# cbacary/MoDeGPT

Measured on AMD Instinct MI355X. Metric: transformer layers compressed/sec (covariance+decomp+rebuild), Llama-3-8B @30%, higher is better.
Workload: dtype f64 from int8 MFMA digit planes, exact route: nine plane pairs + fp64 remainder sums, nothing truncated (error <= 5e-15 per call: fp64 rounding)

## Files before the change

### modegpt_amd/csrc/cov_i8.hip

```cpp
#include <algorithm>
#include <map>
#include <mutex>
#include <tuple>
#include <vector>

#include "common.hpp"
#include <atomic>

namespace mdg {
namespace {

typedef int i32x4 __attribute__((ext_vector_type(4)));
typedef int i32x16 __attribute__((ext_vector_type(16)));

constexpr int NP = 6;
constexpr int TI = 128;
constexpr int KS = 32;
constexpr int PA = TI * KS;
constexpr int FLUSH_STEPS = 2047;
constexpr int TOP_SHIFT = 8 * NP - 10;

constexpr int NSTAT = 8;
constexpr int STAT_D0D1 = 6, STAT_COUNTS = 7;
constexpr int EMAX_COLUMN_OUT = 0x100;

__device__ __forceinline__ void bf16_parts(unsigned b, int& sig, int& ee) {
  const int e = (b >> 7) & 0xFF, m = b & 0x7F;
  sig = e ? (128 | m) : m;
  ee = e ? e : 1;
  if (b & 0x8000) sig = -sig;
}

__global__ __launch_bounds__(256) void i8_colmax_kernel(const bf16_t* x, int64_t ld, int64_t T, int n, int64_t rows_per_block,
                                                        int* emax) {
  const int j = blockIdx.x * 64 + (threadIdx.x & 63);
  const int64_t t0 = (int64_t)blockIdx.y * rows_per_block + (threadIdx.x >> 6);
  const int64_t t1 = min(T, (int64_t)(blockIdx.y + 1) * rows_per_block);
  int best = 1;
  if (j < n)
    for (int64_t t = t0; t < t1; t += 4) {
      int sig, ee;
      bf16_parts(x[t * ld + j], sig, ee);
      if (sig != 0) best = max(best, ee);
    }
  if (j < n) atomicMax(emax + j, best);
}

__device__ __forceinline__ unsigned write_piece_mask(const unsigned (&any)[NP], unsigned char* zmask, int64_t index) {
  unsigned byte = 0;
#pragma unroll
  for (int s = 0; s < NP; s++) {
    const unsigned long long b = __ballot(any[s] != 0);
    const unsigned half = (threadIdx.x & 32) ? (unsigned)(b >> 32) : (unsigned)b;
    byte |= (half != 0) << s;
  }
  if ((threadIdx.x & 31) == 0) zmask[index] = (unsigned char)byte;
  return byte;
// ... 43 lines not shown
          N = (N - d[s]) >> 8;
        }
        d[0] = (int)N;
        dig[0][qq >> 2] |= (unsigned)(d[0] & 255) << (8 * (qq & 3));
#pragma unroll
        for (int s = 0; s < NP; s++) q[s] += d[s] * d[s];
        q[STAT_D0D1] += d[0] * d[1];
      }
#pragma unroll
      for (int s = 0; s < NP; s++) {
        signed char* piece = planes + ((s * groups + G) * (int64_t)nk + kt) * 1024;
        *(i32x4*)(piece + h * 512 + r * 16) = (i32x4){(int)dig[s][0], (int)dig[s][1], (int)dig[s][2], (int)dig[s][3]};
        any[s] |= dig[s][0] | dig[s][1] | dig[s][2] | dig[s][3];
      }
    }
    write_piece_mask(any, zmask, (int64_t)kt * groups + G);
  }
#pragma unroll
  for (int i = 0; i < NSTAT; i++)
    if (q[i]) atomicAdd(&st_lds[i][r], (unsigned long long)q[i]);
  __syncthreads();
  for (int i = threadIdx.x; i < NSTAT * 32; i += 256)
    if (st_lds[i >> 5][i & 31]) atomicAdd(stats + (int64_t)(i >> 5) * n + G * 32 + (i & 31), st_lds[i >> 5][i & 31]);
}

__device__ __forceinline__ int bf16_ee_if_nonzero(unsigned b) {
  const int e = (b >> 7) & 0xFF;
  return (b & 0x7FFF) ? (e ? e : 1) : 0;
}

#ifndef MDG_COLMAX_WGS
#define MDG_COLMAX_WGS 4096
#endif
__global__ __launch_bounds__(256) void i8_colmax_vec_kernel(const bf16_t* x, int64_t ld, int64_t T, int64_t rows_per_block, int* emax) {
  __shared__ int best_lds[128];
  const int cg = threadIdx.x & 15, tl = threadIdx.x >> 4;
  const int j0 = blockIdx.x * 128 + cg * 8;
  const int64_t t0 = (int64_t)blockIdx.y * rows_per_block + tl;
  const int64_t t1 = min(T, (int64_t)(blockIdx.y + 1) * rows_per_block);
  if (threadIdx.x < 128) best_lds[threadIdx.x] = 1;
  __syncthreads();
  int best[8] = {1, 1, 1, 1, 1, 1, 1, 1};
  for (int64_t t = t0; t < t1; t += 16) {
    const i32x4 v = *(const i32x4*)(x + t * ld + j0);
#pragma unroll
    for (int q = 0; q < 4; q++) {
      const unsigned w = (unsigned)v[q];
      best[2 * q] = max(best[2 * q], bf16_ee_if_nonzero(w & 0xFFFF));
      best[2 * q + 1] = max(best[2 * q + 1], bf16_ee_if_nonzero(w >> 16));
    }
  }
#pragma unroll
  for (int q = 0; q < 8; q++) atomicMax(&best_lds[cg * 8 + q], best[q]);
  __syncthreads();
  if (threadIdx.x < 128) atomicMax(emax + blockIdx.x * 128 + threadIdx.x, best_lds[threadIdx.x]);
}

constexpr int SPLIT_TILES = 8;
__global__ __launch_bounds__(256) void i8_split_vec_kernel(const bf16_t* x, int64_t ld, int64_t T, int n, int nk, const int* emax,
                                                           signed char* planes, unsigned long long* stats, unsigned char* zmask) {
  __shared__ __attribute__((aligned(16))) bf16_t tile[64 * 128];
  __shared__ int st_lds[NSTAT + 1][128];
  const int f0 = blockIdx.x * 128;
  const int f = threadIdx.x & 127, ks = threadIdx.x >> 7;
  const int E = emax[f0 + f];
  const int64_t groups = n / 32;
  const int G = (f0 + f) >> 5, r = f & 31;
  for (int i = threadIdx.x; i < (NSTAT + 1) * 128; i += 256) (&st_lds[0][0])[i] = 0;
  int q[NSTAT + 1] = {};
  auto load_tile = [&](int tile_index, i32x4 (&v)[4]) {
    const int64_t tok0 = (int64_t)tile_index * 2 * KS;
#pragma unroll
    for (int c4 = 0; c4 < 4; c4++) {
      const int c = threadIdx.x + 256 * c4;
      const int64_t t = tok0 + (c >> 4);
      v[c4] = (i32x4)0;
      if (t < T) v[c4] = *(const i32x4*)(x + t * ld + f0 + (c & 15) * 8);
    }
  };
  const int tile0 = blockIdx.y * SPLIT_TILES, tiles = (nk + 1) / 2;
  for (int it = 0; it < SPLIT_TILES && tile0 + it < tiles; it++) {
    __syncthreads();
    {
      i32x4 v[4];
      load_tile(tile0 + it, v);
#pragma unroll
      for (int c4 = 0; c4 < 4; c4++) *(i32x4*)(tile + (threadIdx.x + 256 * c4) * 8) = v[c4];
    }
    __syncthreads();
    const int kt = (tile0 + it) * 2 + ks;
    if (kt >= nk) continue;
    unsigned any[NP] = {};
    unsigned deep_dig[2][NP - ALWAYS_WRITTEN_PLANES][4];
#pragma unroll
    for (int h = 0; h < 2; h++) {
      unsigned dig[NP][4];
// ... 98 lines not shown
#pragma unroll
    for (int t = 0; t < NP; t++)
      if (s + t >= P) {
        if (s == t) sq += A[s] * A[t];
        else x += A[s] * A[t];
      }
}
__device__ __forceinline__ double route_violation(const double (&A)[NVAL], int P, double tau_x) {
  double sq, x;
  route_terms(A, P, sq, x);
  return fmax(sq / TAU_SQ, x / tau_x);
}

struct Top2 { double m1; int a1; double m2; };
__device__ __forceinline__ void top2_merge(Top2& a, const Top2& b) {
  if (b.m1 > a.m1 || (b.m1 == a.m1 && b.a1 < a.a1)) {
    a.m2 = fmax(a.m1, b.m2);
    a.m1 = b.m1;
    a.a1 = b.a1;
  } else {
    a.m2 = fmax(a.m2, b.m1);
  }
}

struct RoutePartial {
  Top2 top[NVAL];
  unsigned long long cls[NVAL][64];
  unsigned min_nnz;
};
struct RouteScratch {
  int ticket, forced;
};

__global__ __launch_bounds__(ROUTE_THREADS) void i8_route_kernel(const unsigned long long* __restrict__ stats, int* emax, int n, int64_t n_tokens,
                                                                 double* __restrict__ vals, RoutePartial* partial, RouteScratch* scratch,
                                                                 int* flag, RouteOut* out, int* route_counts, double tolerance) {
  __shared__ unsigned long long group_max[NVAL][64];
  __shared__ Top2 wave_top[ROUTE_THREADS / 64][NVAL];
  __shared__ Top2 top[NVAL];
  __shared__ double floor_of[NVAL];
  __shared__ int decision;
  __shared__ int forced_total, my_ticket;
  __shared__ unsigned min_nnz;
  __shared__ double tau_x_shared;
  const int tid = threadIdx.x, lane = tid & 63, wave = tid >> 6;
  for (int i = tid; i < NVAL * 64; i += ROUTE_THREADS) (&group_max[0][0])[i] = 0ull;
  if (tid == 0) min_nnz = 0xffffffffu;
  __syncthreads();
  auto reduce_top = [&](Top2 (&t)[NVAL]) {
#pragma unroll
    for (int i = 0; i < NVAL; i++) {
#pragma unroll
      for (int off = 32; off >= 1; off >>= 1) {
        Top2 o;
        o.m1 = __shfl_xor(t[i].m1, off);
        o.a1 = __shfl_xor(t[i].a1, off);
        o.m2 = __shfl_xor(t[i].m2, off);
        top2_merge(t[i], o);
      }
      if (lane == 0) wave_top[wave][i] = t[i];
    }
    __syncthreads();
    if (tid < NVAL) {
      Top2 r = wave_top[0][tid];
      for (int w = 1; w < ROUTE_THREADS / 64; w++) top2_merge(r, wave_top[w][tid]);
      top[tid] = r;
    }
    __syncthreads();
  };
// ... 11 lines not shown
      const int ex = emax[j];
      const double nnz = (double)(unsigned)counts, rounded = (double)(unsigned)(counts >> 32);
      const double hi2 = 65536.0 * q[0] + 512.0 * q[STAT_D0D1] + q[1];
      const double norm = (sqrt(fmax(hi2, 0.0)) - 0.5 * sqrt(nnz)) * 4294967296.0;
      const double inv = nnz > 0 ? (norm > 0 ? 1.0 / norm : 1e300) : 0.0;
      double a[NVAL];
#pragma unroll
      for (int s2 = 0; s2 < NP; s2++) a[s2] = q[s2] > 0 ? sqrt(q[s2]) * ldexp(1.0, 8 * (NP - 1 - s2)) * inv : 0.0;
      a[6] = rounded > 0 ? 0.5 * sqrt(rounded) * inv : 0.0;
      nonfinite = (ex & 255) == 255;
      if ((unsigned)counts) atomicMin(&min_nnz, (unsigned)counts);
#pragma unroll
      for (int i = 0; i < NVAL; i++) {
        vals[(int64_t)i * n + j] = a[i];
        if (!nonfinite) t[i] = Top2{a[i], j, -1.0};
      }
      if (nonfinite) emax[j] = ex | EMAX_COLUMN_OUT;
    }
#pragma unroll
    for (int i = 0; i < NVAL; i++)
      if (t[i].m1 > 0.0) atomicMax(&group_max[i][lane], (unsigned long long)__double_as_longlong(t[i].m1));
    const unsigned long long nf = __ballot(nonfinite);
    if (lane == 0 && nf) atomicAdd(&scratch->forced, __popcll(nf));
  }
  reduce_top(t);
  RoutePartial& mine = partial[blockIdx.x];
  if (tid < NVAL) mine.top[tid] = top[tid];
  if (tid == 0) mine.min_nnz = min_nnz;
  for (int i = tid; i < NVAL * 64; i += ROUTE_THREADS) (&mine.cls[0][0])[i] = (&group_max[0][0])[i];
  __threadfence();
  __syncthreads();
  if (tid == 0) my_ticket = atomicAdd(&scratch->ticket, 1);
  __syncthreads();
  if (my_ticket != (int)gridDim.x - 1) return;
  __threadfence();
  const unsigned nwg = gridDim.x;
  if (tid < NVAL) {
    Top2 r = partial[0].top[tid];
    unsigned w = 1;
    for (; w + 4 <= nwg; w += 4) {
      const Top2 b0 = partial[w].top[tid], b1 = partial[w + 1].top[tid], b2 = partial[w + 2].top[tid], b3 = partial[w + 3].top[tid];
      top2_merge(r, b0); top2_merge(r, b1); top2_merge(r, b2); top2_merge(r, b3);
    }
    for (; w < nwg; w++) top2_merge(r, partial[w].top[tid]);
    r.m1 = fmax(r.m1, 0.0);
    r.m2 = fmax(r.m2, 0.0);
    top[tid] = r;
  }
  for (int i = tid; i < NVAL * 64; i += ROUTE_THREADS) {
    unsigned long long m = 0ull;
    unsigned w = 0;
    for (; w + 4 <= nwg; w += 4) {
      const unsigned long long v0 = (&partial[w].cls[0][0])[i], v1 = (&partial[w + 1].cls[0][0])[i], v2 = (&partial[w + 2].cls[0][0])[i],
                               v3 = (&partial[w + 3].cls[0][0])[i];
      m = max(max(m, v0), max(max(v1, v2), v3));
    }
    for (; w < nwg; w++) m = max(m, (&partial[w].cls[0][0])[i]);
    (&group_max[0][0])[i] = m;
  }
  if (tid == 0) {
    forced_total = scratch->forced;
    unsigned m = 0xffffffffu;
    unsigned w = 0;
    for (; w + 4 <= nwg; w += 4) {
      const unsigned v0 = partial[w].min_nnz, v1 = partial[w + 1].min_nnz, v2 = partial[w + 2].min_nnz, v3 = partial[w + 3].min_nnz;
      m = min(min(m, v0), min(min(v1, v2), v3));
    }
    for (; w < nwg; w++) m = min(m, partial[w].min_nnz);
    tau_x_shared = tau_x_of(min(n_tokens, (int64_t)m));
// ... 92 lines not shown
            for (int i = 0; i < NVAL; i++) A2[i] = top[i].a1 == c ? top[i].m2 : top[i].m1;
            const double v = route_violation(A2, P, tau_x);
            if (v < best_v) { best_v = v; best = c; }
          }
          if (best < 0) decision = 1;
          else {
            emax[best] |= EMAX_COLUMN_OUT;
            out->out[n_out] = best;
          }
        }
      }
      __syncthreads();
      const int dec = decision;
      __syncthreads();
      if (dec == 0) return;
      if (dec == 1) break;
      n_out++;
      top_valid = false;
    }
    if (n_out > n_forced) {
      for (int j = tid; j < n; j += ROUTE_THREADS)
        if ((emax[j] & EMAX_COLUMN_OUT) && (emax[j] & 255) != 255) emax[j] &= 255;
      top_valid = false;
      __syncthreads();
    }
  }
  if (tid == 0) {
    out->planes = 0; out->n_out = 0; out->sq = out->x = out->rho = 0.0;
    atomicOr(flag, 2);
  }
  for (int j = tid; j < n; j += ROUTE_THREADS) emax[j] &= 255;
}

__global__ __launch_bounds__(256) void i8_clear_columns_kernel(const RouteOut* route, const int* flag, const int* emax, signed char* planes,
                                                               unsigned char* zmask, int n, int nk) {
  if ((*flag & 2) || (int)blockIdx.x >= route->n_out) return;
  const int j = route->out[blockIdx.x];
  const int64_t groups = n / 32;
  const int G = j >> 5, lane = threadIdx.x & 63, row = lane & 31;
  const bool row_out = (emax[G * 32 + row] & EMAX_COLUMN_OUT) != 0;
  for (int kt = blockIdx.y * 4 + (threadIdx.x >> 6); kt < nk; kt += gridDim.y * 4) {
    const unsigned old_mask = zmask[(int64_t)kt * groups + G];
    unsigned new_mask = 0;
#pragma unroll
    for (int s = 0; s < NP; s++) {
      if (s >= ALWAYS_WRITTEN_PLANES && (old_mask >> s) == 0) continue;
      i32x4* p = (i32x4*)(planes + ((s * groups + G) * (int64_t)nk + kt) * 1024) + lane;
      i32x4 v = *p;
      if (row_out) {
        v = (i32x4)0;
        *p = v;
      }
      if (__ballot((v[0] | v[1] | v[2] | v[3]) != 0)) new_mask |= 1u << s;
    }
    if (lane == 0) zmask[(int64_t)kt * groups + G] = (unsigned char)new_mask;
  }
}

template <int V> struct ic { static constexpr int value = V; };

struct SyrkProblem {
  const signed char* planes;
  const int* emax;
  const unsigned char* zmask;
  double* sigma;
  int64_t ld_sigma;
  int n, block;
};
constexpr int MAX_PROBLEMS = 4;
constexpr int CODE_PROB = 28, CODE_BI = 14;

struct SyrkArgs {
  SyrkProblem prob[MAX_PROBLEMS];
  int nprob, nk;
  unsigned long long* mfma_count;
  const int* route_flag;
  int* route_counts;
  const int2* sched;
  int ngroups;
  double* partial;
  const int4* tail;
  int* xcd_arrive;
  const int* exact_state;
#ifdef MDG_I8_STAMPS
  unsigned long long* stamps;
#endif
#ifdef MDG_I8_WGTIMES
  unsigned long long* wgtimes;
#endif
};
__device__ __forceinline__ int launch_route(const SyrkArgs& a, int& live, int& fallbacks) {
  int six = 0;
  live = fallbacks = 0;
  for (int p = 0; p < a.nprob; p++) {
    const int f = a.route_flag[p];
    if (f & 2) fallbacks++;
    else {
      live++;
      six |= f & 1;
    }
  }
  return live ? six : -1;
// ... 427 lines not shown

constexpr int COMBINE_ELEMS = 1024;
template <int P>
__global__ __launch_bounds__(256) void i8_tail_combine_kernel(SyrkArgs a, int n_tail) {
  constexpr int TJ = wide_tile(P) ? 128 : 64;
  constexpr int PARTS = TI * TJ / COMBINE_ELEMS;
  int live, fallbacks;
  if (!product_launch_runs<P>(a, live, fallbacks)) return;
  const int4 t = a.tail[blockIdx.x / PARTS];
  if (a.route_flag[t.x >> CODE_PROB] & 2) return;
  const SyrkProblem& pr = a.prob[t.x >> CODE_PROB];
  const int bi = (t.x >> CODE_BI) & ((1 << CODE_BI) - 1), bj = t.x & ((1 << CODE_BI) - 1), Q = t.y;
  const double* part = a.partial + (int64_t)t.z * TI * TJ;
#pragma unroll
  for (int i = 0; i < COMBINE_ELEMS / 256; i++) {
    const int e = (blockIdx.x % PARTS) * COMBINE_ELEMS + i * 256 + threadIdx.x;
    const int row = bi * TI + e / TJ, col = bj * TJ + e % TJ;
    if (col > row) continue;
    double* p = pr.sigma + (int64_t)row * pr.ld_sigma + col - (pr.block ? bi * TI : 0);
    double v = *p;
    for (int q = 0; q < Q; q++) v += part[(int64_t)q * TI * TJ + e];
    *p = v;
  }
}

constexpr int COLK_GROUP = 8, COLK_CHUNKS = 64, COLK_WG_COLS = 512, COLK_STAGE = 64, COLK_BATCH = 8;
struct ColArgs {
  const bf16_t* x;
  int64_t ld, T;
  int n, vec;
  const RouteOut* route;
  const int* flag;
  double* part;
};
__device__ __forceinline__ double bf16_bits_to_f64(unsigned b) { return (double)__uint_as_float(b << 16); }

__global__ __launch_bounds__(64) void i8_columns_kernel(ColArgs a) {
  const int pass = blockIdx.z;
  const int n_out = a.route->n_out;
  if ((*a.flag & 2) || pass * COLK_GROUP >= n_out) return;
  const int nj = min(COLK_GROUP, n_out - pass * COLK_GROUP);
  __shared__ __attribute__((aligned(16))) double xj[COLK_STAGE][COLK_GROUP];
  const int lane = threadIdx.x;
  const int my_k = lane % COLK_GROUP;
  const int my_col = my_k < nj ? a.route->out[pass * COLK_GROUP + my_k] : -1;
  const int c0 = blockIdx.x * COLK_WG_COLS + lane * 8;
  const bool active = c0 < a.n;
  const int64_t chunk_len = (a.T + COLK_CHUNKS - 1) / COLK_CHUNKS;
  const int64_t t0 = blockIdx.y * chunk_len, t1 = min(a.T, t0 + chunk_len);
  const unsigned short* xs = (const unsigned short*)a.x;
  auto fetch_group = [&](int64_t t, unsigned short (&g)[COLK_STAGE / 8]) {
#pragma unroll
    for (int i = 0; i < COLK_STAGE / 8; i++) {
      const int64_t tok = t + lane / COLK_GROUP + 8 * i;
      g[i] = (my_col >= 0 && tok < t1) ? xs[tok * a.ld + my_col] : (unsigned short)0;
    }
  };
  double acc[COLK_GROUP][8] = {};
  unsigned short g[COLK_STAGE / 8];
  if (t0 < t1) fetch_group(t0, g);
  for (int64_t t = t0; t < t1; t += COLK_STAGE) {
    __syncthreads();
#pragma unroll
    for (int i = 0; i < COLK_STAGE / 8; i++) xj[lane / COLK_GROUP + 8 * i][my_k] = bf16_bits_to_f64(g[i]);
    __syncthreads();
    if (t + COLK_STAGE < t1) fetch_group(t + COLK_STAGE, g);
    if (!active) continue;
    const int steps = (int)min((int64_t)COLK_STAGE, t1 - t);
    for (int tb = 0; tb < steps; tb += COLK_BATCH) {
      unsigned w[COLK_BATCH][4];
#pragma unroll
      for (int i = 0; i < COLK_BATCH; i++) {
        const bool live = t + tb + i < t1;
// ... 4 lines not shown
        } else {
#pragma unroll
          for (int h = 0; h < 4; h++) w[i][h] = xs[tok * a.ld + c0 + 2 * h] | ((unsigned)xs[tok * a.ld + c0 + 2 * h + 1] << 16);
        }
        if (!live) w[i][0] = w[i][1] = w[i][2] = w[i][3] = 0u;
      }
#pragma unroll
      for (int i = 0; i < COLK_BATCH; i++) {
        double xc[8];
#pragma unroll
        for (int h = 0; h < 4; h++) {
          xc[2 * h] = bf16_bits_to_f64(w[i][h] & 0xFFFFu);
          xc[2 * h + 1] = bf16_bits_to_f64(w[i][h] >> 16);
        }
#pragma unroll
        for (int k = 0; k < COLK_GROUP; k++) {
          const double xk = xj[tb + i][k];
#pragma unroll
          for (int c = 0; c < 8; c++) acc[k][c] += xk * xc[c];
        }
      }
    }
  }
  if (!active) return;
#pragma unroll
  for (int k = 0; k < COLK_GROUP; k++)
    if (k < nj) {
      double* o = a.part + ((int64_t)(pass * COLK_GROUP + k) * COLK_CHUNKS + blockIdx.y) * a.n + c0;
#pragma unroll
      for (int c = 0; c < 8; c++) o[c] = acc[k][c];
    }
}

__global__ __launch_bounds__(256) void i8_columns_reduce_kernel(ColArgs a, const int* emax, double* sigma, int64_t ld_sigma, int block) {
  const int k = blockIdx.y;
  if ((*a.flag & 2) || k >= a.route->n_out) return;
  const int c = blockIdx.x * 256 + threadIdx.x;
  if (c >= a.n) return;
  const int j = a.route->out[k];
  if (block && c / block != j / block) return;
  if ((emax[c] & EMAX_COLUMN_OUT) && c < j) return;
  double v = 0.0;
  for (int q = 0; q < COLK_CHUNKS; q++) v += a.part[((int64_t)k * COLK_CHUNKS + q) * a.n + c];
  const int row = max(c, j), col = min(c, j);
  sigma[(int64_t)row * ld_sigma + col - (block ? row / block * block : 0)] += v;
}


constexpr int LO_CHUNK_STEPS = 64;
constexpr int LO_CAP = 128;
constexpr double LO_ROUND = 8421504.0 / 16777216.0;
constexpr int EXACT_OVERFLOW = 16, EXACT_RAN = 17, EXACT_MODE = 18;
#ifndef MDG_LO_SPARSE_MEAN
#define MDG_LO_SPARSE_MEAN 32
#endif
#ifndef MDG_LO_SPARSE_MAX
#define MDG_LO_SPARSE_MAX 256
#endif
constexpr int LO_SPARSE_MAX = MDG_LO_SPARSE_MAX;
constexpr int LO_SUB = 4, LO_RCAP = 8 * LO_SPARSE_MAX;
constexpr int LO_TILE = 128, LO_PITCH = LO_TILE + 1;

struct __attribute__((aligned(16))) LoEntry {
  double v;
  unsigned off, aux;
};
struct LoProblem {
  const bf16_t* x;
// ... 553 lines not shown
  Schedule sch;
  if (Q >= 2) {
    for (size_t i = 0; i < whole_groups; i++) emit(groups[i]);
    const int pieces = R * Q, tail_rounds = (pieces + 255) / 256;
    std::vector<int2> last((size_t)tail_rounds * 256, make_int2(-1, 0));
    for (int t = 0; t < R; t++) {
      tail.push_back(make_int4(rest[t], Q, t * Q, 0));
      for (int q = 0; q < Q; q++) {
        const int piece = t * Q + q, idx = piece % 256;
        last[(size_t)(piece / 256) * 256 + (idx % 8) * 32 + idx / 8] = make_int2(rest[t], (piece << 10) | (Q << 5) | q);
      }
    }
    table.insert(table.end(), last.begin(), last.end());
    sch.n_tail = (int)tail.size();
    sch.pieces = pieces;
  } else {
    for (auto& g : groups) emit(g);
  }
  sch.ngroups = (int)(table.size() / 32);
  if (hipMalloc((void**)&sch.dev, table.size() * sizeof(int2)) != hipSuccess) return nullptr;
  if (hipMemcpy(sch.dev, table.data(), table.size() * sizeof(int2), hipMemcpyHostToDevice) != hipSuccess) return nullptr;
  if (!tail.empty()) {
    if (hipMalloc((void**)&sch.tail, tail.size() * sizeof(int4)) != hipSuccess) return nullptr;
    if (hipMemcpy(sch.tail, tail.data(), tail.size() * sizeof(int4), hipMemcpyHostToDevice) != hipSuccess) return nullptr;
  }
  return &cache.emplace(key, sch).first->second;
}

constexpr size_t SHARED_BYTES = 256;
struct ProblemWs {
  size_t planes, ints, vals, route, colpart, zmask, lo_entries, lo_counts, lo_xd, lo_rentries, lo_rtotals;
};
int lo_chunks(int64_t T) { return (int)ceil_div(ceil_div(T, (int64_t)KS), (int64_t)LO_CHUNK_STEPS); }
size_t layout(int count, const mdg_cov_problem* pr, ProblemWs* out, size_t* fallback_off) {
  size_t off = SHARED_BYTES + PARTIAL_BYTES, fb = 0;
  for (int i = 0; i < count; i++) {
    const int64_t cols = pr[i].n_feat * pr[i].batch;
    ProblemWs w;
    w.planes = off;
    off += align_up(planes_bytes(pr[i].n_tokens, cols), 256);
    w.ints = off;
    off += align_up(ints_bytes(cols), 256);
    w.vals = off;
    off += align_up((size_t)(NVAL * cols) * sizeof(double) + (size_t)ceil_div(cols, (int64_t)ROUTE_THREADS) * sizeof(RoutePartial), 256);
    w.route = off;
    off += align_up(sizeof(RouteOut), 256);
    w.colpart = off;
    off += align_up((size_t)ROUTE_JMAX * COLK_CHUNKS * (size_t)cols * sizeof(double), 256);
    w.zmask = off;
    off += zmask_bytes(pr[i].n_tokens, cols);
    w.lo_entries = off = align_up(off, 256);
    off += (size_t)cols * lo_chunks(pr[i].n_tokens) * LO_CAP * sizeof(LoEntry);
    w.lo_counts = off;
    off += align_up((size_t)cols * (lo_chunks(pr[i].n_tokens) + 1) * sizeof(int), 256);
    w.lo_xd = off;
    off += align_up((size_t)cols * (size_t)pr[i].n_tokens * sizeof(bf16_t), 256);
    w.lo_rentries = off;
    off += (size_t)(cols / 32) * LO_SUB * LO_RCAP * sizeof(LoEntry);
    w.lo_rtotals = off;
    off += align_up((size_t)(cols / 32) * LO_SUB * sizeof(int), 256);
    if (out) out[i] = w;
    fb = std::max(fb, mdg_cov_accum_ws_bytes(pr[i].n_tokens, pr[i].n_feat, pr[i].batch));
  }
  if (fallback_off) *fallback_off = off;
  return off + fb + 256;
}

bool problems_ok(int count, const mdg_cov_problem* pr) {
  if (count < 1 || count > MAX_PROBLEMS || !pr) return false;
  for (int i = 0; i < count; i++) {
    if (pr[i].n_tokens != pr[0].n_tokens || pr[i].n_tokens < 0 || pr[i].n_tokens >= (1ll << 28) || pr[i].n_feat <= 0 || pr[i].batch < 1) return false;
    if (pr[i].batch == 1 ? pr[i].n_feat % TI != 0 : pr[i].n_feat != TI) return false;
    if (pr[i].n_feat * pr[i].batch >= (1 << 21)) return false;
    if (pr[i].ld < pr[i].n_feat * pr[i].batch || pr[i].ld_sigma < pr[i].n_feat) return false;
    if (pr[i].batch > 1 && (pr[i].ld_sigma != TI || pr[i].sigma_batch_stride != (int64_t)TI * TI)) return false;
// ... 17 lines not shown
  if (have_dev) (void)hipSetDevice(dev0);
  (void)hipGetLastError();
  return rc;
}
}

using namespace mdg;

extern "C" size_t mdg_cov_accum_i8_multi_ws_bytes(int count, const mdg_cov_problem* problems) {
  if (!problems_ok(count, problems) || problems[0].n_tokens == 0) return 0;
  return layout(count, problems, nullptr, nullptr);
}

extern "C" int mdg_cov_accum_i8_multi(int count, const mdg_cov_problem* problems, void* ws, size_t ws_bytes, double tolerance, int flags,
                                      int* used_i8, int* route_counts, void* ev_start, void* ev_stop, void* stream) {
  MDG_CLEAR();
  if (used_i8) *used_i8 = 0;
  MDG_CHECK_ARG(tolerance >= 1.0 && tolerance <= 1e6, "mdg_cov_accum_i8_multi: tolerance factor %g outside [1, 1e6] (1 = guaranteed <= 1.1e-11)",
                tolerance);
  MDG_CHECK_ARG((flags & ~(MDG_I8_NO_EXACT | MDG_I8_EXACT_ALWAYS)) == 0 && flags != (MDG_I8_NO_EXACT | MDG_I8_EXACT_ALWAYS),
                "mdg_cov_accum_i8_multi: bad flags 0x%x", flags);
  bool offer_exact = !(flags & MDG_I8_NO_EXACT);
  for (int i = 0; i < count; i++)
    if ((uint64_t)problems[i].n_tokens * (uint64_t)problems[i].ld * 2ull >= (1ull << 32)) offer_exact = false;
  MDG_CHECK_ARG(problems_ok(count, problems),
                "mdg_cov_accum_i8_multi: 1..%d statistics of the same token count; full ones need n_feat %% 128 == 0, per-head ones "
                "head_dim 128 with contiguous [heads][128][128] sigma; leading dimensions at least the widths (use mdg_cov_accum)",
                MAX_PROBLEMS);
  const int64_t n_tokens = problems[0].n_tokens;
  if (n_tokens == 0) return MDG_OK;
  for (int i = 0; i < count; i++) MDG_CHECK_ARG(problems[i].x && problems[i].sigma, "mdg_cov_accum_i8_multi: null pointer");
  ProblemWs pw[MAX_PROBLEMS];
  size_t fb_off = 0;
  const size_t need = layout(count, problems, pw, &fb_off);
  MDG_CHECK_ARG(ws && ws_bytes >= need, "mdg_cov_accum_i8_multi: workspace %zu < required %zu", ws_bytes, need);
  hipStream_t st = (hipStream_t)stream;
  const int nk = (int)ceil_div(n_tokens, KS);
  int* flag = (int*)ws;
  int* pflag = flag + 12;
  unsigned long long* mfma_count = (unsigned long long*)(flag + 2);
  double* partial = (double*)((char*)ws + SHARED_BYTES);
  void* fb_ws = (char*)ws + fb_off;
  MDG_HIP(hipMemsetAsync(flag, 0, SHARED_BYTES, st));
  SyrkArgs a;
  a.nprob = count;
  a.nk = nk;
  std::vector<std::pair<int, int>> shapes;
  for (int i = 0; i < count; i++) {
    const mdg_cov_problem& q = problems[i];
    const int n = (int)(q.n_feat * q.batch);
    signed char* planes = (signed char*)ws + pw[i].planes;
    int* emax = (int*)((char*)ws + pw[i].ints);
    unsigned long long* stats = (unsigned long long*)(emax + (n + 1) / 2 * 2);
    unsigned char* zmask = (unsigned char*)ws + pw[i].zmask;
    MDG_HIP(hipMemsetAsync(emax, 0, ints_bytes(n), st));
    const bool vec = ((uintptr_t)q.x % 16 == 0) && (q.ld % 8 == 0);
    const int64_t rows_per_block = 2048;
    if (vec) {
      const int64_t slabs = std::min(ceil_div(n_tokens, (int64_t)64), std::max((int64_t)1, (int64_t)MDG_COLMAX_WGS / (n / 128)));
      const int64_t rows_vec = ceil_div(ceil_div(n_tokens, slabs), (int64_t)16) * 16;
      hipLaunchKernelGGL(i8_colmax_vec_kernel, dim3((unsigned)(n / 128), (unsigned)ceil_div(n_tokens, rows_vec)), dim3(256), 0,
                         st, (const bf16_t*)q.x, q.ld, n_tokens, rows_vec, emax);
      hipLaunchKernelGGL(i8_split_vec_kernel, dim3((unsigned)(n / 128), (unsigned)ceil_div(nk, 2 * SPLIT_TILES)), dim3(256), 0, st,
                         (const bf16_t*)q.x, q.ld, n_tokens, n, nk, emax, planes, stats, zmask);
    } else {
      hipLaunchKernelGGL(i8_colmax_kernel, dim3((unsigned)ceil_div(n, 64), (unsigned)ceil_div(n_tokens, rows_per_block)), dim3(256),
                         0, st, (const bf16_t*)q.x, q.ld, n_tokens, n, rows_per_block, emax);
      hipLaunchKernelGGL(i8_split_kernel, dim3((unsigned)(n / 32), (unsigned)ceil_div(nk, SPLIT_STEPS)), dim3(256), 0, st,
                         (const bf16_t*)q.x, q.ld, n_tokens, n, nk, emax, planes, stats, zmask);
    }
    {
      double* vals = (double*)((char*)ws + pw[i].vals);
      RoutePartial* partial = (RoutePartial*)(vals + (size_t)NVAL * n);
      RouteScratch* scratch = (RouteScratch*)(stats + (size_t)NSTAT * n);
      hipLaunchKernelGGL(i8_route_kernel, dim3((unsigned)ceil_div(n, ROUTE_THREADS)), dim3(ROUTE_THREADS), 0, st, stats, emax, n,
                         n_tokens, vals, partial, scratch, pflag + i, (RouteOut*)((char*)ws + pw[i].route), route_counts,
                         tolerance);
    }
    hipLaunchKernelGGL(i8_clear_columns_kernel, dim3(ROUTE_JMAX, (unsigned)std::min(64, (nk + 3) / 4)), dim3(256), 0, st,
                       (const RouteOut*)((char*)ws + pw[i].route), pflag + i, emax, planes, zmask, n, nk);
    MDG_LAUNCH_CHECK();
    a.prob[i] = SyrkProblem{planes, emax, zmask, q.sigma, q.ld_sigma, n, q.batch > 1 ? TI : 0};
    shapes.emplace_back(n / TI, q.batch > 1 ? TI : 0);
  }
  for (int i = count; i < MAX_PROBLEMS; i++) a.prob[i] = a.prob[0];
  a.mfma_count = mfma_count;
  a.route_flag = pflag; a.route_counts = route_counts;
  a.xcd_arrive = flag + 4;
  LoArgs lo;
  a.exact_state = nullptr;
  if (offer_exact) {
    lo.nprob = count;
    lo.nk = nk;
    lo.nch = lo_chunks(n_tokens);
    lo.route_flag = pflag;
    lo.state = flag;
    lo.always = (flags & MDG_I8_EXACT_ALWAYS) ? 1 : 0;
    lo.n_tokens = n_tokens;
    int tiles[3] = {0, 0, 0}, max_groups = 0;
    for (int i = 0; i < count; i++) {
      const mdg_cov_problem& q = problems[i];
      const int n = (int)(q.n_feat * q.batch);
      LoProblem& l = lo.prob[i];
      l.x = (const bf16_t*)q.x; l.ld = q.ld;
      l.planes = a.prob[i].planes; l.zmask = a.prob[i].zmask; l.emax = a.prob[i].emax;
      l.entries = (LoEntry*)((char*)ws + pw[i].lo_entries);
      l.xd = (bf16_t*)((char*)ws + pw[i].lo_xd);
      l.rentries = (LoEntry*)((char*)ws + pw[i].lo_rentries);
      l.rtotals = (int*)((char*)ws + pw[i].lo_rtotals);
      l.pairs = ((uintptr_t)q.x % 4 == 0) && (q.ld % 2 == 0);
      l.counts = (int*)((char*)ws + pw[i].lo_counts);
      l.sigma = q.sigma; l.ld_sigma = q.ld_sigma;
      l.n = n; l.block = q.batch > 1 ? TI : 0;
      const int nG = n / LW_GROUP, per = LW_BLOCK / LW_GROUP;
      for (int tr = 0; tr < 2; tr++) {
        l.tile0[tr] = tiles[tr];
        if (q.batch > 1) {
          tiles[tr] += nG;
        } else {
          for (int P = 0; P * per < nG; P++) tiles[tr] += tr ? std::min(nG, per * (P + 1)) : nG - per * P;
        }
      }
      l.tile0[2] = tiles[2];
      const int rbi = n / TI;
      tiles[2] += q.batch > 1 ? rbi : rbi * (rbi + 1) / 2;
      max_groups = std::max(max_groups, n / 32);
    }
    for (int i = count; i < MAX_PROBLEMS; i++) lo.prob[i] = lo.prob[0];
    for (int k = 0; k < 3; k++) lo.tiles[k] = tiles[k];
    hipLaunchKernelGGL(i8_extract_lo_kernel, dim3((unsigned)max_groups, (unsigned)lo.nch, (unsigned)count), dim3(64), 0, st, lo);
    hipLaunchKernelGGL(i8_compact_lo_kernel, dim3((unsigned)(max_groups * 32), (unsigned)count), dim3(64), 0, st, lo);
    hipLaunchKernelGGL(i8_lo_mode_kernel, dim3(1), dim3(1024), 0, st, lo);
    hipLaunchKernelGGL(i8_residue_lo_kernel, dim3((unsigned)(max_groups * LO_SUB), (unsigned)count), dim3(64), 0, st, lo);
    hipLaunchKernelGGL(i8_copy_xd_kernel, dim3(2048u, (unsigned)count), dim3(256), 0, st, lo);
    hipLaunchKernelGGL(i8_patch_xd_kernel, dim3((unsigned)(max_groups * 32), (unsigned)count), dim3(64), 0, st, lo);
    MDG_LAUNCH_CHECK();
    a.exact_state = flag + EXACT_OVERFLOW;
  }
#ifdef MDG_I8_STAMPS
  static unsigned long long* stamps_dev = nullptr;
  const size_t stamps_n = (size_t)STAMP_WGS * NW * 8;
  if (!stamps_dev) MDG_HIP(hipMalloc(&stamps_dev, stamps_n * 8));
  MDG_HIP(hipMemsetAsync(stamps_dev, 0, stamps_n * 8, st));
  a.stamps = stamps_dev;
#endif
#ifdef MDG_I8_WGTIMES
  static unsigned long long* wg_dev = nullptr;
  if (!wg_dev) MDG_HIP(hipMalloc(&wg_dev, 256 * 64 * 8));
  MDG_HIP(hipMemsetAsync(wg_dev, 0, 256 * 64 * 8, st));
  a.wgtimes = wg_dev;
#endif
  const int n = a.prob[0].n;
  const int rb = n / TI;
  const Schedule* sched_of[2] = {nullptr, nullptr};
  if (rb >= PERSISTENT_MIN_ROWS || count > 1 || problems[0].batch > 1) {
    int dev = 0, n_cu = 0;
    MDG_HIP(hipGetDevice(&dev));
    MDG_HIP(hipDeviceGetAttribute(&n_cu, hipDeviceAttributeMultiprocessorCount, dev));
    if (n_cu == 256)
      for (int i = 0; i < 2; i++) sched_of[i] = schedule_for(shapes, i + 1);
  }
  MDG_CHECK_ARG((count == 1 && problems[0].batch == 1) || (sched_of[0] && sched_of[1]),
                "mdg_cov_accum_i8_multi: several statistics in one launch, and per-head statistics, need the persistent launch (a "
                "256-CU device); use mdg_cov_accum_i8 per full statistic and mdg_cov_accum for the per-head ones");
  {
    size_t zero_bytes = 0;
    for (int i = 0; i < 2; i++)
      if (sched_of[i]) zero_bytes = std::max(zero_bytes, (size_t)sched_of[i]->pieces * TI * (i == 0 ? 128 : 64) * sizeof(double));
    if (zero_bytes) MDG_HIP(hipMemsetAsync(partial, 0, zero_bytes, st));
  }
  a.partial = partial;
  if (ev_start) MDG_HIP(hipEventRecord((hipEvent_t)ev_start, st));
  for (int planes_used : {3, 5, 6}) {
    if (planes_used == 3 && !offer_exact) continue;
    const bool wide = wide_tile(planes_used);
    const int tj = wide ? 128 : 64;
    const size_t lds = (size_t)ring_depth(planes_used) * steps_per_stage(planes_used) * planes_used * (PA + tj * KS);
    const int si = planes_used == 6 ? SB6 : SB5;
    const int sr = (rb + si - 1) / si, nsb = sr * (sr + 1) / 2;
    const int tps = wide ? si * si : 2 * si * si;
    dim3 grid((unsigned)((nsb + 7) / 8 * 8 * tps));
    const Schedule* sch = sched_of[wide ? 0 : 1];
    a.sched = nullptr;
    a.tail = nullptr;
    a.ngroups = 0;
    if (sch) {
      a.sched = sch->dev;
      a.tail = sch->tail;
      a.ngroups = sch->ngroups;
      grid = dim3(256);
    }
    if (planes_used == 3) {
      MDG_HIP(hipFuncSetAttribute((const void*)i8_syrk_kernel<3>, hipFuncAttributeMaxDynamicSharedMemorySize, (int)lds));
      hipLaunchKernelGGL((i8_syrk_kernel<3>), grid, dim3(64 * NW), lds, st, a);
      if (sch && sch->n_tail) hipLaunchKernelGGL((i8_tail_combine_kernel<3>), dim3(sch->n_tail * (TI * tj / COMBINE_ELEMS)), dim3(256), 0, st, a, sch->n_tail);
    } else if (planes_used == 6) {
      MDG_HIP(hipFuncSetAttribute((const void*)i8_syrk_kernel<6>, hipFuncAttributeMaxDynamicSharedMemorySize, (int)lds));
      hipLaunchKernelGGL((i8_syrk_kernel<6>), grid, dim3(64 * NW), lds, st, a);
      if (sch && sch->n_tail) hipLaunchKernelGGL((i8_tail_combine_kernel<6>), dim3(sch->n_tail * (TI * tj / COMBINE_ELEMS)), dim3(256), 0, st, a, sch->n_tail);
    } else {
      MDG_HIP(hipFuncSetAttribute((const void*)i8_syrk_kernel<5>, hipFuncAttributeMaxDynamicSharedMemorySize, (int)lds));
      hipLaunchKernelGGL((i8_syrk_kernel<5>), grid, dim3(64 * NW), lds, st, a);
      if (sch && sch->n_tail) hipLaunchKernelGGL((i8_tail_combine_kernel<5>), dim3(sch->n_tail * (TI * tj / COMBINE_ELEMS)), dim3(256), 0, st, a, sch->n_tail);
    }
    MDG_LAUNCH_CHECK();
  }
  if (ev_stop) MDG_HIP(hipEventRecord((hipEvent_t)ev_stop, st));
  if (offer_exact) {
    const size_t lds = (size_t)LO_TILE * LO_PITCH * sizeof(double);
    MDG_HIP(hipFuncSetAttribute((const void*)i8_lo_product_kernel, hipFuncAttributeMaxDynamicSharedMemorySize, (int)lds));
    hipLaunchKernelGGL(i8_lo_product_kernel, dim3((unsigned)lo.tiles[2]), dim3(LO_THREADS), lds, st, lo);
    hipLaunchKernelGGL(i8_lo_wide_kernel<false>, dim3((unsigned)lo.tiles[0]), dim3(LO_THREADS), 0, st, lo);
    hipLaunchKernelGGL(i8_lo_wide_kernel<true>, dim3((unsigned)lo.tiles[1]), dim3(LO_THREADS), 0, st, lo);
    MDG_LAUNCH_CHECK();
  }
  for (int i = 0; i < count; i++) {
    const mdg_cov_problem& q = problems[i];
    const int n = (int)(q.n_feat * q.batch);
    ColArgs c;
    c.x = (const bf16_t*)q.x; c.ld = q.ld; c.T = n_tokens; c.n = n;
    c.vec = ((uintptr_t)q.x % 16 == 0) && (q.ld % 8 == 0);
    c.route = (const RouteOut*)((char*)ws + pw[i].route);
    c.flag = pflag + i;
    c.part = (double*)((char*)ws + pw[i].colpart);
    hipLaunchKernelGGL(i8_columns_kernel, dim3((unsigned)ceil_div(n, COLK_WG_COLS), COLK_CHUNKS, ROUTE_JMAX / COLK_GROUP), dim3(64), 0, st, c);
    hipLaunchKernelGGL(i8_columns_reduce_kernel, dim3((unsigned)ceil_div(n, 256), ROUTE_JMAX), dim3(256), 0, st, c, a.prob[i].emax, q.sigma,
                       q.ld_sigma, q.batch > 1 ? TI : 0);
    MDG_LAUNCH_CHECK();
  }
  for (int i = 0; i < count; i++) {
    const mdg_cov_problem& q = problems[i];
    const int fb = cov_accum_gated(q.x, MDG_BF16, n_tokens, q.n_feat, q.batch, q.ld, 0, q.sigma, q.ld_sigma, q.sigma_batch_stride, fb_ws,
                                   ws_bytes - fb_off, pflag + i, 2, 2, stream);
    if (fb != MDG_OK) return fb;
  }
#ifdef MDG_I8_STAMPS
  {
    static unsigned long long host[STAMP_WGS * NW * 8];
    MDG_HIP(hipMemcpyAsync(host, a.stamps, sizeof(host), hipMemcpyDeviceToHost, st));
    MDG_HIP(hipStreamSynchronize(st));
    double sum[2][6] = {};
    long cnt[2] = {};
    for (int w = 0; w < STAMP_WGS * NW; w++) {
      const unsigned long long* o = host + (size_t)w * 8;
      if (!o[6]) continue;
      const int role = (w % NW) >= NW / 2;
      for (int i = 0; i < 6; i++) sum[role][i] += (double)o[i] / (double)o[6];
      cnt[role]++;
    }
    for (int role = 0; role < 2; role++)
      if (cnt[role])
        fprintf(stderr, "[stamps n=%d] waves %s: per k-step cycles (s_memtime): wait+barrier %.0f  refill-first %.0f  reads+mfma-issue %.0f  "
                        "wait+refill-last %.0f  | whole tile / nk %.0f  mfma/step %.1f  (%ld waves)\n", n, role ? "4-7" : "0-3",
                sum[role][0] / cnt[role], sum[role][1] / cnt[role], sum[role][2] / cnt[role], sum[role][3] / cnt[role],
                sum[role][4] / cnt[role], sum[role][5] / cnt[role], cnt[role]);
  }
#endif
#ifdef MDG_I8_WGTIMES
  {
    static unsigned long long host[256 * 64];
// ... 103 lines not shown
```

Before: 1.178.

## Batch per-problem preprocessing kernels into single multi-problem launches and merge memsets

```diff
diff --git a/modegpt_amd/csrc/cov_i8.hip b/modegpt_amd/csrc/cov_i8.hip
--- a/modegpt_amd/csrc/cov_i8.hip
+++ b/modegpt_amd/csrc/cov_i8.hip
@@ -23,6 +23,35 @@
 constexpr int NSTAT = 8;
 constexpr int STAT_D0D1 = 6, STAT_COUNTS = 7;
 constexpr int EMAX_COLUMN_OUT = 0x100;
+constexpr int MAX_PROBLEMS = 4;
+
+struct RouteOut;
+struct RoutePartial;
+struct RouteScratch;
+struct CallProblem {
+  const bf16_t* x;
+  int64_t ld;
+  int n, cb0;
+  int* emax;
+  unsigned long long* stats;
+  signed char* planes;
+  unsigned char* zmask;
+  double* vals;
+  RoutePartial* rpartial;
+  RouteScratch* scratch;
+  RouteOut* route;
+  int* flag;
+};
+struct CallArgs {
+  CallProblem prob[MAX_PROBLEMS];
+  int nprob, nk;
+  int64_t T;
+};
+__device__ __forceinline__ int call_problem_of_block(const CallArgs& a, int cb) {
+  int p = 0;
+  while (p + 1 < a.nprob && cb >= a.prob[p + 1].cb0) p++;
+  return p;
+}
 
 __device__ __forceinline__ void bf16_parts(unsigned b, int& sig, int& ee) {
   const int e = (b >> 7) & 0xFF, m = b & 0x7F;
@@ -132,10 +161,14 @@
 #ifndef MDG_COLMAX_WGS
 #define MDG_COLMAX_WGS 4096
 #endif
-__global__ __launch_bounds__(256) void i8_colmax_vec_kernel(const bf16_t* x, int64_t ld, int64_t T, int64_t rows_per_block, int* emax) {
+__global__ __launch_bounds__(256) void i8_colmax_vec_kernel(CallArgs a, int64_t rows_per_block) {
+  const CallProblem& pr = a.prob[call_problem_of_block(a, blockIdx.x)];
+  const bf16_t* x = pr.x;
+  const int64_t ld = pr.ld, T = a.T;
+  const int cb = blockIdx.x - pr.cb0;
   __shared__ int best_lds[128];
   const int cg = threadIdx.x & 15, tl = threadIdx.x >> 4;
-  const int j0 = blockIdx.x * 128 + cg * 8;
+  const int j0 = cb * 128 + cg * 8;
   const int64_t t0 = (int64_t)blockIdx.y * rows_per_block + tl;
   const int64_t t1 = min(T, (int64_t)(blockIdx.y + 1) * rows_per_block);
   if (threadIdx.x < 128) best_lds[threadIdx.x] = 1;
@@ -153,15 +186,22 @@
 #pragma unroll
   for (int q = 0; q < 8; q++) atomicMax(&best_lds[cg * 8 + q], best[q]);
   __syncthreads();
-  if (threadIdx.x < 128) atomicMax(emax + blockIdx.x * 128 + threadIdx.x, best_lds[threadIdx.x]);
+  if (threadIdx.x < 128) atomicMax(pr.emax + cb * 128 + threadIdx.x, best_lds[threadIdx.x]);
 }
 
 constexpr int SPLIT_TILES = 8;
-__global__ __launch_bounds__(256) void i8_split_vec_kernel(const bf16_t* x, int64_t ld, int64_t T, int n, int nk, const int* emax,
-                                                           signed char* planes, unsigned long long* stats, unsigned char* zmask) {
+__global__ __launch_bounds__(256) void i8_split_vec_kernel(CallArgs a) {
+  const CallProblem& pr = a.prob[call_problem_of_block(a, blockIdx.x)];
+  const bf16_t* x = pr.x;
+  const int64_t ld = pr.ld, T = a.T;
+  const int n = pr.n, nk = a.nk;
+  const int* emax = pr.emax;
+  signed char* planes = pr.planes;
+  unsigned long long* stats = pr.stats;
+  unsigned char* zmask = pr.zmask;
   __shared__ __attribute__((aligned(16))) bf16_t tile[64 * 128];
   __shared__ int st_lds[NSTAT + 1][128];
-  const int f0 = blockIdx.x * 128;
+  const int f0 = (blockIdx.x - pr.cb0) * 128;
   const int f = threadIdx.x & 127, ks = threadIdx.x >> 7;
   const int E = emax[f0 + f];
   const int64_t groups = n / 32;
@@ -326,9 +366,19 @@
   int ticket, forced;
 };
 
-__global__ __launch_bounds__(ROUTE_THREADS) void i8_route_kernel(const unsigned long long* __restrict__ stats, int* emax, int n, int64_t n_tokens,
-                                                                 double* __restrict__ vals, RoutePartial* partial, RouteScratch* scratch,
-                                                                 int* flag, RouteOut* out, int* route_counts, double tolerance) {
+__global__ __launch_bounds__(ROUTE_THREADS) void i8_route_kernel(CallArgs a, int* route_counts, double tolerance) {
+  const CallProblem& pr = a.prob[blockIdx.y];
+  const int n = pr.n;
+  const unsigned nwg = (unsigned)((n + ROUTE_THREADS - 1) / ROUTE_THREADS);
+  if (blockIdx.x >= nwg) return;
+  const int64_t n_tokens = a.T;
+  const unsigned long long* __restrict__ stats = pr.stats;
+  int* emax = pr.emax;
+  double* __restrict__ vals = pr.vals;
+  RoutePartial* partial = pr.rpartial;
+  RouteScratch* scratch = pr.scratch;
+  int* flag = pr.flag;
+  RouteOut* out = pr.route;
   __shared__ unsigned long long group_max[NVAL][64];
   __shared__ Top2 wave_top[ROUTE_THREADS / 64][NVAL];
   __shared__ Top2 top[NVAL];
@@ -406,9 +456,8 @@
   __syncthreads();
   if (tid == 0) my_ticket = atomicAdd(&scratch->ticket, 1);
   __syncthreads();
-  if (my_ticket != (int)gridDim.x - 1) return;
+  if (my_ticket != (int)nwg - 1) return;
   __threadfence();
-  const unsigned nwg = gridDim.x;
   if (tid < NVAL) {
     Top2 r = partial[0].top[tid];
     unsigned w = 1;
@@ -567,9 +616,14 @@
   for (int j = tid; j < n; j += ROUTE_THREADS) emax[j] &= 255;
 }
 
-__global__ __launch_bounds__(256) void i8_clear_columns_kernel(const RouteOut* route, const int* flag, const int* emax, signed char* planes,
-                                                               unsigned char* zmask, int n, int nk) {
-  if ((*flag & 2) || (int)blockIdx.x >= route->n_out) return;
+__global__ __launch_bounds__(256) void i8_clear_columns_kernel(CallArgs a) {
+  const CallProblem& pr = a.prob[blockIdx.z];
+  const RouteOut* route = pr.route;
+  const int* emax = pr.emax;
+  signed char* planes = pr.planes;
+  unsigned char* zmask = pr.zmask;
+  const int n = pr.n, nk = a.nk;
+  if ((*pr.flag & 2) || (int)blockIdx.x >= route->n_out) return;
   const int j = route->out[blockIdx.x];
   const int64_t groups = n / 32;
   const int G = j >> 5, lane = threadIdx.x & 63, row = lane & 31;
@@ -602,7 +656,6 @@
   int64_t ld_sigma;
   int n, block;
 };
-constexpr int MAX_PROBLEMS = 4;
 constexpr int CODE_PROB = 28, CODE_BI = 14;
 
 struct SyrkArgs {
@@ -1096,13 +1149,22 @@
   const RouteOut* route;
   const int* flag;
   double* part;
+  const int* emax;
+  double* sigma;
+  int64_t ld_sigma;
+  int block;
 };
+struct ColMulti {
+  ColArgs c[MAX_PROBLEMS];
+};
+constexpr int COLK_PASSES = ROUTE_JMAX / COLK_GROUP;
 __device__ __forceinline__ double bf16_bits_to_f64(unsigned b) { return (double)__uint_as_float(b << 16); }
 
-__global__ __launch_bounds__(64) void i8_columns_kernel(ColArgs a) {
-  const int pass = blockIdx.z;
+__global__ __launch_bounds__(64) void i8_columns_kernel(ColMulti m) {
+  const ColArgs& a = m.c[blockIdx.z / COLK_PASSES];
+  const int pass = blockIdx.z % COLK_PASSES;
   const int n_out = a.route->n_out;
-  if ((*a.flag & 2) || pass * COLK_GROUP >= n_out) return;
+  if ((*a.flag & 2) || pass * COLK_GROUP >= n_out || (int)blockIdx.x * COLK_WG_COLS >= a.n) return;
   const int nj = min(COLK_GROUP, n_out - pass * COLK_GROUP);
   __shared__ __attribute__((aligned(16))) double xj[COLK_STAGE][COLK_GROUP];
   const int lane = threadIdx.x;
@@ -1173,8 +1235,13 @@
     }
 }
 
-__global__ __launch_bounds__(256) void i8_columns_reduce_kernel(ColArgs a, const int* emax, double* sigma, int64_t ld_sigma, int block) {
-  const int k = blockIdx.y;
+__global__ __launch_bounds__(256) void i8_columns_reduce_kernel(ColMulti m) {
+  const ColArgs& a = m.c[blockIdx.y / ROUTE_JMAX];
+  const int k = blockIdx.y % ROUTE_JMAX;
+  const int* emax = a.emax;
+  double* sigma = a.sigma;
+  const int64_t ld_sigma = a.ld_sigma;
+  const int block = a.block;
   if ((*a.flag & 2) || k >= a.route->n_out) return;
   const int c = blockIdx.x * 256 + threadIdx.x;
   if (c >= a.n) return;
@@ -1794,15 +1861,21 @@
   size_t planes, ints, vals, route, colpart, zmask, lo_entries, lo_counts, lo_xd, lo_rentries, lo_rtotals;
 };
 int lo_chunks(int64_t T) { return (int)ceil_div(ceil_div(T, (int64_t)KS), (int64_t)LO_CHUNK_STEPS); }
-size_t layout(int count, const mdg_cov_problem* pr, ProblemWs* out, size_t* fallback_off) {
-  size_t off = SHARED_BYTES + PARTIAL_BYTES, fb = 0;
+size_t layout(int count, const mdg_cov_problem* pr, ProblemWs* out, size_t* fallback_off, size_t* partial_off = nullptr) {
+  if (count < 1 || count > MAX_PROBLEMS) return 0;
+  size_t off = SHARED_BYTES, fb = 0;
+  ProblemWs ws[MAX_PROBLEMS];
+  for (int i = 0; i < count; i++) {
+    ws[i].ints = off;
+    off += align_up(ints_bytes(pr[i].n_feat * pr[i].batch), 256);
+  }
+  if (partial_off) *partial_off = off;
+  off += PARTIAL_BYTES;
   for (int i = 0; i < count; i++) {
     const int64_t cols = pr[i].n_feat * pr[i].batch;
-    ProblemWs w;
+    ProblemWs& w = ws[i];
     w.planes = off;
     off += align_up(planes_bytes(pr[i].n_tokens, cols), 256);
-    w.ints = off;
-    off += align_up(ints_bytes(cols), 256);
     w.vals = off;
     off += align_up((size_t)(NVAL * cols) * sizeof(double) + (size_t)ceil_div(cols, (int64_t)ROUTE_THREADS) * sizeof(RoutePartial), 256);
     w.route = off;
@@ -1886,58 +1959,101 @@
   for (int i = 0; i < count; i++) MDG_CHECK_ARG(problems[i].x && problems[i].sigma, "mdg_cov_accum_i8_multi: null pointer");
   ProblemWs pw[MAX_PROBLEMS];
   size_t fb_off = 0;
-  const size_t need = layout(count, problems, pw, &fb_off);
+  size_t partial_off = 0;
+  const size_t need = layout(count, problems, pw, &fb_off, &partial_off);
   MDG_CHECK_ARG(ws && ws_bytes >= need, "mdg_cov_accum_i8_multi: workspace %zu < required %zu", ws_bytes, need);
   hipStream_t st = (hipStream_t)stream;
   const int nk = (int)ceil_div(n_tokens, KS);
   int* flag = (int*)ws;
   int* pflag = flag + 12;
   unsigned long long* mfma_count = (unsigned long long*)(flag + 2);
-  double* partial = (double*)((char*)ws + SHARED_BYTES);
+  double* partial = (double*)((char*)ws + partial_off);
   void* fb_ws = (char*)ws + fb_off;
-  MDG_HIP(hipMemsetAsync(flag, 0, SHARED_BYTES, st));
   SyrkArgs a;
   a.nprob = count;
   a.nk = nk;
   std::vector<std::pair<int, int>> shapes;
+  CallArgs c;
+  c.nprob = count;
+  c.nk = nk;
+  c.T = n_tokens;
+  int vec_blocks = 0;
+  bool all_vec = true;
   for (int i = 0; i < count; i++) {
     const mdg_cov_problem& q = problems[i];
     const int n = (int)(q.n_feat * q.batch);
-    signed char* planes = (signed char*)ws + pw[i].planes;
-    int* emax = (int*)((char*)ws + pw[i].ints);
-    unsigned long long* stats = (unsigned long long*)(emax + (n + 1) / 2 * 2);
-    unsigned char* zmask = (unsigned char*)ws + pw[i].zmask;
-    MDG_HIP(hipMemsetAsync(emax, 0, ints_bytes(n), st));
+    CallProblem& cp = c.prob[i];
+    cp.x = (const bf16_t*)q.x;
+    cp.ld = q.ld;
+    cp.n = n;
+    cp.cb0 = vec_blocks;
+    cp.planes = (signed char*)ws + pw[i].planes;
+    cp.emax = (int*)((char*)ws + pw[i].ints);
+    cp.stats = (unsigned long long*)(cp.emax + (n + 1) / 2 * 2);
+    cp.zmask = (unsigned char*)ws + pw[i].zmask;
+    cp.vals = (double*)((char*)ws + pw[i].vals);
+    cp.rpartial = (RoutePartial*)(cp.vals + (size_t)NVAL * n);
+    cp.scratch = (RouteScratch*)(cp.stats + (size_t)NSTAT * n);
+    cp.route = (RouteOut*)((char*)ws + pw[i].route);
+    cp.flag = pflag + i;
     const bool vec = ((uintptr_t)q.x % 16 == 0) && (q.ld % 8 == 0);
-    const int64_t rows_per_block = 2048;
-    if (vec) {
-      const int64_t slabs = std::min(ceil_div(n_tokens, (int64_t)64), std::max((int64_t)1, (int64_t)MDG_COLMAX_WGS / (n / 128)));
-      const int64_t rows_vec = ceil_div(ceil_div(n_tokens, slabs), (int64_t)16) * 16;
-      hipLaunchKernelGGL(i8_colmax_vec_kernel, dim3((unsigned)(n / 128), (unsigned)ceil_div(n_tokens, rows_vec)), dim3(256), 0,
-                         st, (const bf16_t*)q.x, q.ld, n_tokens, rows_vec, emax);
-      hipLaunchKernelGGL(i8_split_vec_kernel, dim3((unsigned)(n / 128), (unsigned)ceil_div(nk, 2 * SPLIT_TILES)), dim3(256), 0, st,
-                         (const bf16_t*)q.x, q.ld, n_tokens, n, nk, emax, planes, stats, zmask);
-    } else {
-      hipLaunchKernelGGL(i8_colmax_kernel, dim3((unsigned)ceil_div(n, 64), (unsigned)ceil_div(n_tokens, rows_per_block)), dim3(256),
-                         0, st, (const bf16_t*)q.x, q.ld, n_tokens, n, rows_per_block, emax);
-      hipLaunchKernelGGL(i8_split_kernel, dim3((unsigned)(n / 32), (unsigned)ceil_div(nk, SPLIT_STEPS)), dim3(256), 0, st,
-                         (const bf16_t*)q.x, q.ld, n_tokens, n, nk, emax, planes, stats, zmask);
-    }
-    {
-      double* vals = (double*)((char*)ws + pw[i].vals);
-      RoutePartial* partial = (RoutePartial*)(vals + (size_t)NVAL * n);
-      RouteScratch* scratch = (RouteScratch*)(stats + (size_t)NSTAT * n);
-      hipLaunchKernelGGL(i8_route_kernel, dim3((unsigned)ceil_div(n, ROUTE_THREADS)), dim3(ROUTE_THREADS), 0, st, stats, emax, n,
-                         n_tokens, vals, partial, scratch, pflag + i, (RouteOut*)((char*)ws + pw[i].route), route_counts,
-                         tolerance);
-    }
-    hipLaunchKernelGGL(i8_clear_columns_kernel, dim3(ROUTE_JMAX, (unsigned)std::min(64, (nk + 3) / 4)), dim3(256), 0, st,
-                       (const RouteOut*)((char*)ws + pw[i].route), pflag + i, emax, planes, zmask, n, nk);
-    MDG_LAUNCH_CHECK();
-    a.prob[i] = SyrkProblem{planes, emax, zmask, q.sigma, q.ld_sigma, n, q.batch > 1 ? TI : 0};
+    all_vec = all_vec && vec;
+    if (vec) vec_blocks += n / 128;
+    a.prob[i] = SyrkProblem{cp.planes, cp.emax, cp.zmask, q.sigma, q.ld_sigma, n, q.batch > 1 ? TI : 0};
     shapes.emplace_back(n / TI, q.batch > 1 ? TI : 0);
   }
-  for (int i = count; i < MAX_PROBLEMS; i++) a.prob[i] = a.prob[0];
+  for (int i = count; i < MAX_PROBLEMS; i++) {
+    a.prob[i] = a.prob[0];
+    c.prob[i] = c.prob[0];
+  }
+  const int n0 = a.prob[0].n;
+  const int rb = n0 / TI;
+  const Schedule* sched_of[2] = {nullptr, nullptr};
+  if (rb >= PERSISTENT_MIN_ROWS || count > 1 || problems[0].batch > 1) {
+    int dev = 0, n_cu = 0;
+    MDG_HIP(hipGetDevice(&dev));
+    MDG_HIP(hipDeviceGetAttribute(&n_cu, hipDeviceAttributeMultiprocessorCount, dev));
+    if (n_cu == 256)
+      for (int i = 0; i < 2; i++) sched_of[i] = schedule_for(shapes, i + 1);
+  }
+  MDG_CHECK_ARG((count == 1 && problems[0].batch == 1) || (sched_of[0] && sched_of[1]),
+                "mdg_cov_accum_i8_multi: several statistics in one launch, and per-head statistics, need the persistent launch (a "
+                "256-CU device); use mdg_cov_accum_i8 per full statistic and mdg_cov_accum for the per-head ones");
+  {
+    size_t zero_bytes = 0;
+    for (int i = 0; i < 2; i++)
+      if (sched_of[i]) zero_bytes = std::max(zero_bytes, (size_t)sched_of[i]->pieces * TI * (i == 0 ? 128 : 64) * sizeof(double));
+    MDG_HIP(hipMemsetAsync(ws, 0, partial_off + zero_bytes, st));
+  }
+  if (vec_blocks) {
+    const int64_t slabs = std::min(ceil_div(n_tokens, (int64_t)64), std::max((int64_t)1, (int64_t)MDG_COLMAX_WGS / vec_blocks));
+    const int64_t rows_vec = ceil_div(ceil_div(n_tokens, slabs), (int64_t)16) * 16;
+    CallArgs cv = c;
+    cv.nprob = 0;
+    for (int i = 0; i < count; i++)
+      if (((uintptr_t)problems[i].x % 16 == 0) && (problems[i].ld % 8 == 0)) cv.prob[cv.nprob++] = c.prob[i];
+    for (int i = cv.nprob; i < MAX_PROBLEMS; i++) cv.prob[i] = cv.prob[0];
+    hipLaunchKernelGGL(i8_colmax_vec_kernel, dim3((unsigned)vec_blocks, (unsigned)ceil_div(n_tokens, rows_vec)), dim3(256), 0, st, cv,
+                       rows_vec);
+    hipLaunchKernelGGL(i8_split_vec_kernel, dim3((unsigned)vec_blocks, (unsigned)ceil_div(nk, 2 * SPLIT_TILES)), dim3(256), 0, st, cv);
+  }
+  if (!all_vec)
+    for (int i = 0; i < count; i++) {
+      const mdg_cov_problem& q = problems[i];
+      if (((uintptr_t)q.x % 16 == 0) && (q.ld % 8 == 0)) continue;
+      const CallProblem& cp = c.prob[i];
+      const int64_t rows_per_block = 2048;
+      hipLaunchKernelGGL(i8_colmax_kernel, dim3((unsigned)ceil_div(cp.n, 64), (unsigned)ceil_div(n_tokens, rows_per_block)), dim3(256),
+                         0, st, cp.x, cp.ld, n_tokens, cp.n, rows_per_block, cp.emax);
+      hipLaunchKernelGGL(i8_split_kernel, dim3((unsigned)(cp.n / 32), (unsigned)ceil_div(nk, SPLIT_STEPS)), dim3(256), 0, st, cp.x, cp.ld,
+                         n_tokens, cp.n, nk, cp.emax, cp.planes, cp.stats, cp.zmask);
+    }
+  int max_n = 0;
+  for (int i = 0; i < count; i++) max_n = std::max(max_n, c.prob[i].n);
+  hipLaunchKernelGGL(i8_route_kernel, dim3((unsigned)ceil_div(max_n, ROUTE_THREADS), (unsigned)count), dim3(ROUTE_THREADS), 0, st, c,
+                     route_counts, tolerance);
+  hipLaunchKernelGGL(i8_clear_columns_kernel, dim3(ROUTE_JMAX, (unsigned)std::min(64, (nk + 3) / 4), (unsigned)count), dim3(256), 0, st, c);
+  MDG_LAUNCH_CHECK();
   a.mfma_count = mfma_count;
   a.route_flag = pflag; a.route_counts = route_counts;
   a.xcd_arrive = flag + 4;
@@ -2004,25 +2120,6 @@
   MDG_HIP(hipMemsetAsync(wg_dev, 0, 256 * 64 * 8, st));
   a.wgtimes = wg_dev;
 #endif
-  const int n = a.prob[0].n;
-  const int rb = n / TI;
-  const Schedule* sched_of[2] = {nullptr, nullptr};
-  if (rb >= PERSISTENT_MIN_ROWS || count > 1 || problems[0].batch > 1) {
-    int dev = 0, n_cu = 0;
-    MDG_HIP(hipGetDevice(&dev));
-    MDG_HIP(hipDeviceGetAttribute(&n_cu, hipDeviceAttributeMultiprocessorCount, dev));
-    if (n_cu == 256)
-      for (int i = 0; i < 2; i++) sched_of[i] = schedule_for(shapes, i + 1);
-  }
-  MDG_CHECK_ARG((count == 1 && problems[0].batch == 1) || (sched_of[0] && sched_of[1]),
-                "mdg_cov_accum_i8_multi: several statistics in one launch, and per-head statistics, need the persistent launch (a "
-                "256-CU device); use mdg_cov_accum_i8 per full statistic and mdg_cov_accum for the per-head ones");
-  {
-    size_t zero_bytes = 0;
-    for (int i = 0; i < 2; i++)
-      if (sched_of[i]) zero_bytes = std::max(zero_bytes, (size_t)sched_of[i]->pieces * TI * (i == 0 ? 128 : 64) * sizeof(double));
-    if (zero_bytes) MDG_HIP(hipMemsetAsync(partial, 0, zero_bytes, st));
-  }
   a.partial = partial;
   if (ev_start) MDG_HIP(hipEventRecord((hipEvent_t)ev_start, st));
   for (int planes_used : {3, 5, 6}) {
@@ -2068,18 +2165,25 @@
     hipLaunchKernelGGL(i8_lo_wide_kernel<true>, dim3((unsigned)lo.tiles[1]), dim3(LO_THREADS), 0, st, lo);
     MDG_LAUNCH_CHECK();
   }
-  for (int i = 0; i < count; i++) {
-    const mdg_cov_problem& q = problems[i];
-    const int n = (int)(q.n_feat * q.batch);
-    ColArgs c;
-    c.x = (const bf16_t*)q.x; c.ld = q.ld; c.T = n_tokens; c.n = n;
-    c.vec = ((uintptr_t)q.x % 16 == 0) && (q.ld % 8 == 0);
-    c.route = (const RouteOut*)((char*)ws + pw[i].route);
-    c.flag = pflag + i;
-    c.part = (double*)((char*)ws + pw[i].colpart);
-    hipLaunchKernelGGL(i8_columns_kernel, dim3((unsigned)ceil_div(n, COLK_WG_COLS), COLK_CHUNKS, ROUTE_JMAX / COLK_GROUP), dim3(64), 0, st, c);
-    hipLaunchKernelGGL(i8_columns_reduce_kernel, dim3((unsigned)ceil_div(n, 256), ROUTE_JMAX), dim3(256), 0, st, c, a.prob[i].emax, q.sigma,
-                       q.ld_sigma, q.batch > 1 ? TI : 0);
+  {
+    ColMulti cm;
+    for (int i = 0; i < count; i++) {
+      const mdg_cov_problem& q = problems[i];
+      ColArgs& ca = cm.c[i];
+      ca.x = (const bf16_t*)q.x; ca.ld = q.ld; ca.T = n_tokens; ca.n = c.prob[i].n;
+      ca.vec = ((uintptr_t)q.x % 16 == 0) && (q.ld % 8 == 0);
+      ca.route = c.prob[i].route;
+      ca.flag = pflag + i;
+      ca.part = (double*)((char*)ws + pw[i].colpart);
+      ca.emax = a.prob[i].emax;
+      ca.sigma = q.sigma;
+      ca.ld_sigma = q.ld_sigma;
+      ca.block = q.batch > 1 ? TI : 0;
+    }
+    for (int i = count; i < MAX_PROBLEMS; i++) cm.c[i] = cm.c[0];
+    hipLaunchKernelGGL(i8_columns_kernel, dim3((unsigned)ceil_div(max_n, COLK_WG_COLS), COLK_CHUNKS, (unsigned)(COLK_PASSES * count)), dim3(64), 0,
+                       st, cm);
+    hipLaunchKernelGGL(i8_columns_reduce_kernel, dim3((unsigned)ceil_div(max_n, 256), (unsigned)(ROUTE_JMAX * count)), dim3(256), 0, st, cm);
     MDG_LAUNCH_CHECK();
   }
   for (int i = 0; i < count; i++) {
```

New measurement: 1.184 (median of 6 runs). No clear change (+0.5%).
